# kyutai-labs/pocket-tts

Measured on AMD Instinct MI355X. Metric: audio-seconds/sec (xRT), 100M en model, whole job over all GPUs, higher is better.
Workload: dtype f32

## Files before the change

### include/ptts.h

```cpp
#ifndef PTTS_H_
#define PTTS_H_

#include <stdint.h>

#ifdef __cplusplus
extern "C" {
#endif

#define PTTS_ABI_VERSION 1

typedef struct ptts_engine ptts_engine;
typedef struct ptts_lm_state ptts_lm_state;
typedef struct ptts_mimi_state ptts_mimi_state;
typedef struct ptts_graph ptts_graph;
typedef struct ptts_resampler ptts_resampler;
typedef struct ptts_stretcher ptts_stretcher;

typedef struct ptts_config {
  int32_t d_model, num_heads, num_layers, ff_dim, ldim;
  int32_t flow_dim, flow_depth;
  float max_period;
  int32_t m_dim, m_heads, m_layers, m_ff, m_context;
  float m_max_period;
  int32_t n_filters, ratios[3], kernel_size, res_kernel_size, last_kernel_size, compress;
// ... 109 lines not shown
int ptts_copy_to_host_async(ptts_engine *e, void *h_dst, const void *d_src, int64_t bytes, void *stream);
int ptts_timer_start(ptts_engine *e, void *stream);
int ptts_timer_stop_ms(ptts_engine *e, void *stream, float *h_ms);
int64_t ptts_debug_read(ptts_engine *e, void *state, int32_t is_mimi, const char *name, float *d_out,
                        int64_t capacity, int32_t *rows, int32_t *cols, void *stream);
typedef struct ptts_gemm_case {
  int32_t M, N, C, ntaps;
  int32_t T, xstride, halo, halo_mode;
  int32_t wfmt, pre, epi, act;
  int32_t cfg;
  int32_t krot, lds_target;
  const float *x, *x_prev;
  const float *w, *bias;
  const float *ln_w, *ln_b;
  const float *prevec;
  const float *mod_shift, *mod_scale;
  const float *r, *g, *ls;
  float *y;
  float *w_eff, *w_eff_lo;
  float *ln_s, *ln_c;
  char *label;
  int32_t label_cap;
  int32_t cfg_used;
} ptts_gemm_case;
int ptts_debug_gemm(ptts_engine *e, ptts_gemm_case *c, void *stream);
typedef struct ptts_codec_gemm_case {
  int32_t M, N, C, ntaps;
  int32_t T, halo, par;
  int32_t fmt, kind, pre, epi, act, cfg;
  int32_t mode, cout, stride;
  int32_t yf8, H, Tq, ring, cap;
  float xs, yinv;
  const float *x, *x_prev;
  const float *w, *bias, *ln_w, *ln_b;
  const float *r, *ls;
  const int32_t *offset;
  float *y, *yraw, *y_i16;
  float *x_eff, *xp_eff;
  float *w_eff, *wscale;
  float *ln_s, *ln_c, *rope;
  char *label;
  int32_t label_cap;
  int32_t cfg_used;
} ptts_codec_gemm_case;
int ptts_debug_codec_gemm(ptts_engine *e, ptts_codec_gemm_case *c, void *stream);
typedef struct ptts_attn_case {
// ... 26 lines not shown
```

### pocket_tts_amd/_lib.py

```python

from __future__ import annotations

import ctypes as C
import os
import subprocess
from pathlib import Path

PKG = Path(__file__).resolve().parent
LIB_PATH = PKG / "libptts.so"
SRC = PKG / "csrc" / "ptts.hip"
HEADER = PKG.parent / "include" / "ptts.h"

HIPCC_FLAGS = ["--offload-arch=gfx950", "-O3", "-std=c++17", "-ffp-contract=on", "-Wno-unused-value", "-Wno-unused-result",
               "-shared", "-fPIC"]


class PttsConfig(C.Structure):
    _fields_ = [
        ("d_model", C.c_int32), ("num_heads", C.c_int32), ("num_layers", C.c_int32), ("ff_dim", C.c_int32),
        ("ldim", C.c_int32), ("flow_dim", C.c_int32), ("flow_depth", C.c_int32), ("max_period", C.c_float),
        ("m_dim", C.c_int32), ("m_heads", C.c_int32), ("m_layers", C.c_int32), ("m_ff", C.c_int32),
        ("m_context", C.c_int32), ("m_max_period", C.c_float),
        ("n_filters", C.c_int32), ("ratios", C.c_int32 * 3), ("kernel_size", C.c_int32),
        ("res_kernel_size", C.c_int32), ("last_kernel_size", C.c_int32), ("compress", C.c_int32),
        ("upsample_stride", C.c_int32),
    ]


class PttsTensor(C.Structure):
    _fields_ = [("name", C.c_char_p), ("d_data", C.c_void_p), ("numel", C.c_int64)]


class PttsGemmCase(C.Structure):
    _fields_ = [
        *[(f, C.c_int32) for f in ("M", "N", "C", "ntaps", "T", "xstride", "halo", "halo_mode", "wfmt", "pre", "epi", "act",
                                   "cfg", "krot", "lds_target")],
        *[(f, C.c_void_p) for f in ("x", "x_prev", "w", "bias", "ln_w", "ln_b", "prevec", "mod_shift", "mod_scale", "r", "g",
                                    "ls", "y", "w_eff", "w_eff_lo", "ln_s", "ln_c")],
        ("label", C.c_void_p), ("label_cap", C.c_int32), ("cfg_used", C.c_int32),
    ]


class PttsCodecGemmCase(C.Structure):
    _fields_ = [
        *[(f, C.c_int32) for f in ("M", "N", "C", "ntaps", "T", "halo", "par", "fmt", "kind", "pre", "epi", "act", "cfg",
                                   "mode", "cout", "stride", "yf8", "H", "Tq", "ring", "cap")],
        ("xs", C.c_float), ("yinv", C.c_float),
        *[(f, C.c_void_p) for f in ("x", "x_prev", "w", "bias", "ln_w", "ln_b", "r", "ls", "offset", "y", "yraw", "y_i16",
                                    "x_eff", "xp_eff", "w_eff", "wscale", "ln_s", "ln_c", "rope", "label")],
        ("label_cap", C.c_int32), ("cfg_used", C.c_int32),
    ]


class PttsAttnCase(C.Structure):
    _fields_ = [
        *[(f, C.c_int32) for f in ("B", "Tq", "H", "T", "cap", "ring", "ctx", "splits", "h16", "layer", "n_pre", "pre_T",
                                   "pre_cap", "cascade", "kernel")],
        ("poison_k", C.c_float), ("poison_v", C.c_float),
        *[(f, C.c_void_p) for f in ("q", "k", "v", "pk", "pv", "offset", "pre_len", "pre_id", "y", "label")],
        ("label_cap", C.c_int32), ("kernel_used", C.c_int32), ("splits_used", C.c_int32),
    ]

# ... 165 lines not shown
```

### pocket_tts_amd/csrc/ptts.hip

```cpp
#include "ptts_host.h"
#include "ptts_flow.h"
#include "ptts_bf16.h"
#include "ptts_lm.h"

#include <algorithm>
#include <array>
#include <cmath>
#include <cstdio>
#include <cstring>

static thread_local std::string g_err;
int fail(int code, const std::string &msg) {
  g_err = msg;
  return code;
}
static thread_local std::string g_launch_err;
bool launch_err_pending() { return !g_launch_err.empty(); }
int take_launch_err() {
  std::string m;
  m.swap(g_launch_err);
  return fail(-4, m);
}
void note_launch_err(const std::string &msg) { if (g_launch_err.empty()) g_launch_err = msg; }

// ... 1719 lines not shown

extern "C" void ptts_mimi_state_destroy(ptts_mimi_state *s) {
  if (!s) return;
  hipSetDevice(s->e->device);
  hipDeviceSynchronize();
  hipFree(s->frame); hipFree(s->offset); hipFree(s->kv); hipFree(s->zl); hipFree(s->zq); hipFree(s->u0);
  hipFree(s->u); hipFree(s->h); hipFree(s->ao); hipFree(s->ff); hipFree(s->q); hipFree(s->part);
  hipFree(s->tr_out); hipFree(s->a0); hipFree(s->pcm_dbg); hipFree(s->pcm_part); hipFree(s->pcm_carry); hipFree(s->rope);
  for (int i = 0; i < 3; ++i) { hipFree(s->cbuf[i]); hipFree(s->craw[i]); hipFree(s->rbuf[i]); hipFree(s->sbuf[i]); }
  delete s;
}

extern "C" int ptts_mimi_state_reset(ptts_mimi_state *s, void *stream) {
  hipStream_t st = S(s->e, stream);
  HIPCHK(hipMemsetAsync(s->frame, 0, sizeof(int), st));
  HIPCHK(hipMemsetAsync(s->offset, 0, s->B * sizeof(int), st));
  HIPCHK(hipMemsetAsync(s->zq, 0, (size_t)2 * s->zq_stride * 4, st));
  HIPCHK(hipMemsetAsync(s->tr_out, 0, (size_t)2 * s->tr_stride * 4, st));
  HIPCHK(hipMemsetAsync(s->a0, 0, (size_t)2 * s->a0_stride * 4, st));
  for (int i = 0; i < 3; ++i) {
    HIPCHK(hipMemsetAsync(s->cbuf[i], 0, (size_t)2 * s->c_stride[i] * 4, st));
    HIPCHK(hipMemsetAsync(s->sbuf[i], 0, (size_t)2 * s->s_stride[i] * 4, st));
  }
  HIPCHK(hipMemsetAsync(s->kv, 0, (size_t)s->e->cfg.m_layers * 2 * s->kv_plane() * 4, st));
  if (s->pcm_carry) HIPCHK(hipMemsetAsync(s->pcm_carry, 0, (size_t)2 * s->pcm_cstride * 4, st));
  s->h_frame = 0;
  return 0;
}

extern "C" int ptts_mimi_state_reset_row(ptts_mimi_state *s, int32_t row, void *stream) {
  if (!s || row < 0 || row >= s->B) return fail(-1, "reset_row: row out of range");
  hipStream_t st = S(s->e, stream);
  const int CF = s->e->cfg.m_dim / 16;
  const bool h16 = s->e->codec_bf16, f8 = s->e->codec_fp8;
  const int e_tr = h16 ? 2 : 4, e_a0 = f8 ? 1 : h16 ? 2 : 4;
  set_int_kernel<<<1, 64, 0, st>>>(s->offset + row, 1, 0);
  auto zero_block = [&](float *buf, long stride_floats, int par, int esz) -> hipError_t {
    const size_t per_seq = (size_t)stride_floats / s->B;
    return hipMemsetAsync((char *)buf + (size_t)par * stride_floats * 4 + (size_t)row * per_seq * esz, 0, per_seq * esz, st);
  };
  for (int par = 0; par < 2; ++par) {
    zero_row_fm_kernel<<<cdiv(CF * 16, 256), 256, 0, st>>>(s->zq + par * s->zq_stride, CF, row);
    HIPCHK(zero_block(s->tr_out, s->tr_stride, par, e_tr));
    HIPCHK(zero_block(s->a0, s->a0_stride, par, e_a0));
    for (int i = 0; i < 3; ++i) {
      HIPCHK(zero_block(s->cbuf[i], s->c_stride[i], par, e_a0));
      HIPCHK(zero_block(s->sbuf[i], s->s_stride[i], par, (f8 && i == 2) ? 2 : e_a0));
// ... 755 lines not shown
```

### pocket_tts_amd/csrc/ptts_debug.hip

```cpp
#include "ptts_bf16.h"
#include "ptts_host.h"

#include <algorithm>
#include <cstring>


static constexpr unsigned kDbgUnwritten = 0x7fc00000u;
static constexpr unsigned kDbgGuard = 0x7fa5a5a5u;
static constexpr long kDbgGuardFloats = 16384;
static constexpr long kAttnGuard = 16 * 64;

static __global__ void dbg_guard_kernel(const unsigned *p, long n, unsigned pattern, int *bad) {
  const long i = (long)blockIdx.x * blockDim.x + threadIdx.x;
  if (i < n && p[i] != pattern) atomicOr(bad, 1);
}
__device__ __forceinline__ float dbg_e4m3(uint8_t b) { return __builtin_amdgcn_cvt_f32_fp8((int)b, 0); }
static __global__ void dbg_from_codec_kernel(const void *src, float *dst, int M, int N, int KB, int fmt) {
  const long i = (long)blockIdx.x * blockDim.x + threadIdx.x;
  if (i >= (long)M * N) return;
  const int m = i / N, n = i - (long)m * N;
  const size_t o = fmh_off(m, n & ~3, KB) + (n & 3);
  dst[i] = fmt == 0 ? (float)((const __bf16 *)src)[o] : dbg_e4m3(((const uint8_t *)src)[o]);
}

// ... 104 lines not shown
  const long i = (long)blockIdx.x * blockDim.x + threadIdx.x;
  if (i >= (long)M * N) return;
  const int m = i / N, n = i - (long)m * N;
  dst[i] = src[(((size_t)(m >> 4) * NF + (n >> 4)) * 64 + 16 * ((n & 15) >> 2) + (m & 15)) * 4 + (n & 3)];
}
static __global__ void dbg_unpack_weight_kernel(const void *img, const float *scale, int fmt, float *dst, int N, int KF) {
  const long K = (long)KF * 16;
  const long i = (long)blockIdx.x * blockDim.x + threadIdx.x;
  if (i >= (long)N * K) return;
  const int n = i / K, k = i - (long)n * K;
  const int nt = n >> 4, kf = k >> 4, j = k & 3, lane = 16 * ((k & 15) >> 2) + (n & 15);
  float v;
  if (fmt == 0) v = ((const float *)img)[(((size_t)nt * KF + kf) * 64 + lane) * 4 + j];
  else if (fmt == 1) v = ((float)((const uint8_t *)img)[(size_t)nt * KF * 256 + (size_t)(kf >> 2) * 1024 + lane * 16 + 4 * (kf & 3) + j] - 128.f) * scale[n];
  else v = (float)((const __bf16 *)img)[(((size_t)nt * (KF / 2) + (kf >> 1)) * 64 + lane) * 8 + (kf & 1) * 4 + j];
  dst[i] = v;
}

static int debug_gemm(ptts_engine *e, ptts_gemm_case *c, hipStream_t st, ptts_engine &scr) {
  const int M = c->M, N = c->N, C = c->C, ntaps = c->ntaps, pre = c->pre;
  c->cfg_used = -1;
  if (!c->x || !c->w || !c->y) return fail(-1, "debug_gemm: x, w and y are required");
  if (M < 1 || N < 1 || C < 16 || C % 16 || ntaps < 1) return fail(-1, "debug_gemm: bad shape");
  if (c->wfmt < 0 || c->wfmt > 3 || pre < PRE_NONE || pre > PRE_LNMOD || c->epi < EPI_STORE || c->epi > EPI_GATE ||
      c->act < ACT_NONE || c->act > ACT_ELU || c->cfg < -1 || c->cfg >= kNumCfg)
    return fail(-1, "debug_gemm: enumeration out of range");
  if (c->lds_target < 0 || c->lds_target > 64 * 1024) return fail(-1, "debug_gemm: lds_target above 64 KB");
  int rows_in = M;
  if (ntaps > 1) {
    if (c->T < 16 || c->T % 16 || M % c->T || c->xstride < 1 || c->halo < 0 || c->halo > c->T * c->xstride ||
        ntaps - 1 - c->halo >= c->xstride || c->halo_mode < 0 || c->halo_mode > 2 || (c->halo_mode == 0 && !c->x_prev))
      return fail(-1, "debug_gemm: bad convolution geometry");
    if (pre == PRE_LNFOLD || pre == PRE_LNMOD || pre == PRE_ADDSILU) return fail(-1, "debug_gemm: per-channel prologues are for Linear layers");
    rows_in = M * c->xstride;
  } else if (c->xstride != 1) {
    return fail(-1, "debug_gemm: a Linear has xstride 1");
  }
  if ((pre == PRE_LNFOLD && (!c->ln_w || !c->ln_b)) || (pre == PRE_ADDSILU && !c->prevec) ||
      (pre == PRE_LNMOD && (!c->mod_shift || !c->mod_scale || !c->ln_w != !c->ln_b)))
    return fail(-1, "debug_gemm: missing prologue operand");
  if ((c->epi == EPI_RES && !c->r) || (c->epi == EPI_GATE && (!c->r || !c->g))) return fail(-1, "debug_gemm: missing epilogue operand");
  if (c->wfmt >= 2 && (C / 16) * ntaps % 2) return fail(-1, "debug_gemm: bf16 images need an even number of k-fragments");

  const ptts_tensor tw{"w", c->w, (int64_t)N * C * ntaps}, tb{"b", c->bias, N}, tg{"ln_w", c->ln_w, C}, tbe{"ln_b", c->ln_b, C};
  scr.tmap["w"] = &tw;
  if (c->bias) scr.tmap["b"] = &tb;
  if (pre == PRE_LNFOLD) { scr.tmap["ln_w"] = &tg; scr.tmap["ln_b"] = &tbe; }
  Lin L;
  const bool fold = pre == PRE_LNFOLD;
  CHK(pack_lin(&scr, &L, {{"w", c->bias ? "b" : "", N}}, C, ntaps, 0, 0, 0, fold ? "ln_w" : "", fold ? "ln_b" : "", 0,
// ... 18 lines not shown
    CHK(dallocT(&scr, out, (size_t)pad));
    HIPCHK(hipMemcpyAsync(*out, src, (size_t)n * 4, hipMemcpyDeviceToDevice, st));
    return 0;
  };
  const long yfl = (long)MT * NT * 256;
  float *yfm = nullptr;
  CHK(dallocT(&scr, &yfm, yfl + kDbgGuardFloats));
  HIPCHK(hipMemsetD32Async((hipDeviceptr_t)yfm, (int)kDbgUnwritten, yfl, st));
  HIPCHK(hipMemsetD32Async((hipDeviceptr_t)(yfm + yfl), (int)kDbgGuard, kDbgGuardFloats, st));

  GemmArgs a = mk_gemm(L, xfm, CF, MT, M);
  if (c->wfmt == 3) { a.Wq = (const uint8_t *)L.wsh; a.W = (const float *)L.wsl; a.wfmt = 3; }
  a.Xdstride = xfl;
  a.T = ntaps > 1 ? c->T : 16;
  a.xstride = c->xstride;
  a.halo = c->halo;
  a.halo_mode = c->halo_mode;
  a.zeros = e->zeros;
  a.krot = c->krot;
  a.epi = c->epi;
  a.act = c->act;
  a.Y = yfm;
  a.YF = NT;
  float *tmp = nullptr;
  if (pre == PRE_ADDSILU) { CHK(copy_pad(c->prevec, C, C, &tmp)); a.prevec = tmp; }
  if (pre == PRE_LNMOD) {
    if (c->ln_w) {
      CHK(copy_pad(c->ln_w, C, C, &tmp)); a.lnm_w = tmp;
      CHK(copy_pad(c->ln_b, C, C, &tmp)); a.lnm_b = tmp;
    }
    CHK(to_fm(c->mod_shift, M, C, MT, CF, &tmp)); a.mod_shift = tmp;
    CHK(to_fm(c->mod_scale, M, C, MT, CF, &tmp)); a.mod_scale = tmp;
    a.modF = CF;
  }
  if (c->epi == EPI_RES || c->epi == EPI_GATE) { CHK(to_fm(c->r, M, N, MT, NT, &tmp)); a.R = tmp; a.RF = NT; }
  if (c->epi == EPI_GATE) { CHK(to_fm(c->g, M, N, MT, NT, &tmp)); a.G = tmp; a.GF = NT; }
  if (c->epi == EPI_RES && c->ls) { CHK(copy_pad(c->ls, N, NT * 16, &tmp)); a.ls = tmp; }

  KnobScope knobs(c->lds_target, c->krot);
  int cfg = c->cfg;
  if (cfg >= 0 ? !(pre_supported(a.wfmt, pre) && cfg_valid(cfg, a, pre)) : (cfg = choose_cfg(st, a, pre)) < 0) {
    HIPCHK(hipStreamSynchronize(st));
    return 1;
  }
  std::string label;
  launch_gemm_cfg(st, a, pre, cfg, &label);
  LAUNCHCHK();
  c->cfg_used = cfg;
  put_label(label, c->label, c->label_cap);
  dbg_from_fm_kernel<<<cdiv((long)M * N, 256), 256, 0, st>>>(yfm, c->y, M, N, NT);
  const long nk = (long)N * L.KF * 16;
  if (c->w_eff) {
    if (c->wfmt == 0) dbg_unpack_weight_kernel<<<cdiv(nk, 256), 256, 0, st>>>(L.w, nullptr, 0, c->w_eff, N, L.KF);
    else if (c->wfmt == 1) dbg_unpack_weight_kernel<<<cdiv(nk, 256), 256, 0, st>>>(L.wq, L.wscale, 1, c->w_eff, N, L.KF);
    else dbg_unpack_weight_kernel<<<cdiv(nk, 256), 256, 0, st>>>(c->wfmt == 2 ? L.wb16 : L.wsh, nullptr, 2, c->w_eff, N, L.KF);
  }
  if (c->w_eff_lo && c->wfmt == 3) dbg_unpack_weight_kernel<<<cdiv(nk, 256), 256, 0, st>>>(L.wsl, nullptr, 2, c->w_eff_lo, N, L.KF);
  if (fold && c->ln_s) HIPCHK(hipMemcpyAsync(c->ln_s, L.ln_s, (size_t)N * 4, hipMemcpyDeviceToDevice, st));
  if (fold && c->ln_c) HIPCHK(hipMemcpyAsync(c->ln_c, L.ln_c, (size_t)N * 4, hipMemcpyDeviceToDevice, st));
  return check_guards(scr, st, {yfm + yfl}, kDbgGuardFloats, "debug_gemm: " + label + " wrote past its output");
}

extern "C" int ptts_debug_gemm(ptts_engine *e, ptts_gemm_case *c, void *stream) {
  if (!e || !c) return fail(-1, "debug_gemm: null argument");
  return run_case(e, stream, [&](hipStream_t st, ptts_engine &scr) { return debug_gemm(e, c, st, scr); });
}


static __global__ void dbg_attn_q_kernel(const float *q, float *Q, int B, int Tq, int H, int QB, float poison) {
  const long i = (long)blockIdx.x * blockDim.x + threadIdx.x;
  if (i >= (long)B * H * QB * 1024) return;
  const int j = i & 3, lane = (i >> 2) & 63, df = (i >> 8) & 3;
  const long r = i >> 10;
// ... 384 lines not shown
```

### pocket_tts_amd/csrc/ptts_dispatch.hip

```cpp
#include "ptts_host.h"
#include "ptts_bf16.h"

#include <algorithm>
#include <cstdio>
#include <cstring>

template <int TN, int TM, int WK, int WN, int WM>
static void launch_cfg_q8(hipStream_t st, const GemmArgs &a, int pre) {
  dim3 grid(cdiv(a.NT, TN * WN), cdiv(a.MT, TM * WM));
  dim3 block(64 * WK * WN * WM);
  if (pre == PRE_LNFOLD) gemm_kernel<TN, TM, WK, WN, WM, PRE_LNFOLD, true><<<grid, block, 0, st>>>(a);
  else gemm_kernel<TN, TM, WK, WN, WM, PRE_NONE, true><<<grid, block, 0, st>>>(a);
}

static thread_local int g_lds_target = 0;
static unsigned lds_pad(int static_bytes) { return g_lds_target > static_bytes ? (unsigned)(g_lds_target - static_bytes) : 0u; }
#define LDS_LAUNCH(kernel, grid, block, dyn, st, arg) (kernel)<<<(grid), (block), (dyn), (st)>>>(arg)

template <int TN, int TM, int WK, int WN, int WM>
static void launch_cfg(hipStream_t st, const GemmArgs &a, int pre) {
  dim3 grid(cdiv(a.NT, TN * WN), cdiv(a.MT, TM * WM), pre == PRE_ADDSILU_ROW ? std::max(1, a.row_nz) : 1);
  dim3 block(64 * WK * WN * WM);
  const unsigned dyn = lds_pad(WK > 1 ? WK * WN * WM * TN * TM * 1024 : 0);
  switch (pre) {
    case PRE_NONE: LDS_LAUNCH((gemm_kernel<TN, TM, WK, WN, WM, PRE_NONE>), grid, block, dyn, st, a); break;
    case PRE_LNFOLD: LDS_LAUNCH((gemm_kernel<TN, TM, WK, WN, WM, PRE_LNFOLD>), grid, block, dyn, st, a); break;
    case PRE_LNMOD: LDS_LAUNCH((gemm_kernel<TN, TM, WK, WN, WM, PRE_LNMOD>), grid, block, dyn, st, a); break;
    case PRE_ELU: LDS_LAUNCH((gemm_kernel<TN, TM, WK, WN, WM, PRE_ELU>), grid, block, dyn, st, a); break;
    case PRE_ADDSILU_ROW: LDS_LAUNCH((gemm_kernel<TN, TM, WK, WN, WM, PRE_ADDSILU_ROW>), grid, block, dyn, st, a); break;
    case PRE_LNMOD_ROW: LDS_LAUNCH((gemm_kernel<TN, TM, WK, WN, WM, PRE_LNMOD_ROW>), grid, block, dyn, st, a); break;
    default: LDS_LAUNCH((gemm_kernel<TN, TM, WK, WN, WM, PRE_ADDSILU>), grid, block, dyn, st, a); break;
  }
}

template <int BMT, int BNT>
static void launch_lds(hipStream_t st, const GemmArgs &a, int pre) {
  dim3 grid(cdiv(a.NT, BNT), cdiv(a.MT, BMT));
  static const int variant = [] { const char *v = getenv("PTTS_LDS_VARIANT"); return v ? atoi(v) : 1; }();
  if constexpr (BMT == 4 && BNT <= 4) {
    if (variant == 1 && g_lds_target) {
      const unsigned dyn3 = lds_pad(3 * (BMT + BNT) * 2 * 1024);
      if (pre == PRE_LNFOLD) gemm_lds_kernel<BMT, BNT, 2, PRE_LNFOLD, 3><<<grid, 256, dyn3, st>>>(a);
      else if (pre == PRE_ELU) gemm_lds_kernel<BMT, BNT, 2, PRE_ELU, 3><<<grid, 256, dyn3, st>>>(a);
      else gemm_lds_kernel<BMT, BNT, 2, PRE_NONE, 3><<<grid, 256, dyn3, st>>>(a);
      return;
    }
    if (variant == 2 && g_lds_target && a.KF % 4 == 0 && pre != PRE_ELU) {
      const unsigned dyn4 = lds_pad(2 * (BMT + BNT) * 4 * 1024);
      if (pre == PRE_LNFOLD) gemm_lds_kernel<BMT, BNT, 4, PRE_LNFOLD><<<grid, 256, dyn4, st>>>(a);
      else gemm_lds_kernel<BMT, BNT, 4, PRE_NONE><<<grid, 256, dyn4, st>>>(a);
      return;
    }
  }
  const unsigned dyn = lds_pad(2 * (BMT + BNT) * 2 * 1024);
  if (pre == PRE_LNFOLD) LDS_LAUNCH((gemm_lds_kernel<BMT, BNT, 2, PRE_LNFOLD>), grid, dim3(256), dyn, st, a);
  else if (pre == PRE_ELU) LDS_LAUNCH((gemm_lds_kernel<BMT, BNT, 2, PRE_ELU>), grid, dim3(256), dyn, st, a);
  else LDS_LAUNCH((gemm_lds_kernel<BMT, BNT, 2, PRE_NONE>), grid, dim3(256), dyn, st, a);
}

static int pick_cfg(const GemmArgs &a) {
  const long tiled = (long)cdiv(a.NT, 4) * cdiv(a.MT, 8);
  if (a.MT >= 256 && a.NT >= 4 && a.KF % 2 == 0 && a.epi != EPI_QKV && !a.mod_scale) return a.NT >= 8 ? 8 : 9;
  if (a.MT > 4 && tiled >= 192) return a.NT >= 4 ? 3 : a.NT >= 2 ? 4 : 5;
  if (a.MT >= 8 && a.NT >= 2 && a.KF >= 32 && (long)cdiv(a.NT, 2) * cdiv(a.MT, 4) >= 128) return 7;
  if (a.MT > 64) {
    if (tiled < 192) return 6;
    return a.NT >= 4 ? 3 : a.NT >= 2 ? 4 : 5;
  }
  int tm = a.MT >= 4 ? 4 : a.MT >= 2 ? 2 : 1;
  while (tm > 1 && (long)a.NT * cdiv(a.MT, tm) < 256) tm >>= 1;
  return tm == 4 ? 2 : tm == 2 ? 1 : 0;
}
static const char *const kCfgName[kNumCfg] = {
    "gemm<1,1,8,1,1>", "gemm<1,2,4,1,1>", "gemm<1,4,4,1,1>", "gemm<2,4,1,2,2>", "gemm<2,4,1,1,4>", "gemm<1,4,1,1,4>",
    "gemm<1,1,1,1,4>", "gemm<2,4,4,1,1>", "gemm_lds<4,8,2>", "gemm_lds<4,4,2>", "gemm<2,2,4,1,1>", "gemm<1,1,4,1,1>",
    "gemm_lds<4,2,2>", "gemm<1,2,1,2,2>", "gemm<2,4,2,2,1>", "gemm_lds<8,8,2>", "gemm_lds<8,4,2>", "gemm_lds<8,2,2>"};
static const int kCfgShape[kNumCfg][5] = {{1, 1, 8, 1, 1}, {1, 2, 4, 1, 1}, {1, 4, 4, 1, 1}, {2, 4, 1, 2, 2}, {2, 4, 1, 1, 4},
                                          {1, 4, 1, 1, 4}, {1, 1, 1, 1, 4}, {2, 4, 4, 1, 1}, {8, 4, 0, 0, 0}, {4, 4, 0, 0, 0},
                                          {2, 2, 4, 1, 1}, {1, 1, 4, 1, 1}, {2, 4, 0, 0, 0}, {1, 2, 1, 2, 2}, {2, 4, 2, 2, 1},
                                          {8, 8, 0, 0, 0}, {4, 8, 0, 0, 0}, {2, 8, 0, 0, 0}};

static bool q8_cfg(int cfg) { return cfg == 0 || cfg == 1 || cfg == 2 || cfg == 3 || cfg == 7 || cfg == 10 || cfg == 11; }
static bool b16_cfg(int cfg) { return cfg != 0 && q8_cfg(cfg); }

bool cfg_valid(int cfg, const GemmArgs &a, int pre) {
  const int *s = kCfgShape[cfg];
  if (a.wfmt == 3) {
    if (!split_cfg(cfg) || (pre != PRE_NONE && pre != PRE_LNFOLD)) return false;
    if (a.KF % (2 * s[2])) return false;
  } else if (a.wfmt) {
    if (!(a.wfmt == 2 ? b16_cfg(cfg) : q8_cfg(cfg)) || (pre != PRE_NONE && pre != PRE_LNFOLD)) return false;
    if (a.KF % ((a.wfmt == 1 ? 4 : 2) * s[2])) return false;
  }
  if (s[2] == 0) {
    if (a.KF % 2 || (pre != PRE_NONE && pre != PRE_LNFOLD && pre != PRE_ELU)) return false;
    return a.MT >= s[1] && 2 * a.NT >= s[0];
  }
  const int tn = s[0] * s[3], tm = s[1] * s[4];
  if (tm > 1 && tm > 2 * a.MT) return false;
  if (tn > 1 && tn > 2 * a.NT) return false;
  if (s[2] > 1 && a.KF < 2) return false;
  return true;
}

static int swz_for(int cfg, const GemmArgs &a) {
  static const int swz_env = [] { const char *v = getenv("PTTS_SWZ"); return v ? atoi(v) : -1; }();
  const int *sh = kCfgShape[cfg];
  const int gx = sh[2] == 0 ? cdiv(a.NT, sh[0]) : cdiv(a.NT, sh[0] * sh[3]);
  if (gx <= 1) return 0;
  return swz_env >= 0 ? swz_env : ((double)a.M * a.CF > (double)a.NT * 16 * a.KF && a.MT >= 64);
}

static void launch_by_cfg(hipStream_t st, const GemmArgs &a_in, int pre, int cfg) {
  GemmArgs a = a_in;
  a.swz = swz_for(cfg, a);
  if (a.wfmt == 2) {
    launch_gemm_b16(st, a, pre, cfg, 0);
    return;
  }
  if (a.wfmt == 3) {
    const int *sh = kCfgShape[cfg];
    launch_gemm_split(st, a, pre, cfg, lds_pad(sh[2] > 1 ? sh[2] * sh[3] * sh[4] * sh[0] * sh[1] * 1024 : 0));
// ... 9 lines not shown
      case 11: launch_cfg_q8<1, 1, 4, 1, 1>(st, a, pre); break;
      default: launch_cfg_q8<2, 4, 1, 2, 2>(st, a, pre); break;
    }
    return;
  }
  switch (cfg) {
    case 0: launch_cfg<1, 1, 8, 1, 1>(st, a, pre); break;
    case 1: launch_cfg<1, 2, 4, 1, 1>(st, a, pre); break;
    case 2: launch_cfg<1, 4, 4, 1, 1>(st, a, pre); break;
    case 3: launch_cfg<2, 4, 1, 2, 2>(st, a, pre); break;
    case 4: launch_cfg<2, 4, 1, 1, 4>(st, a, pre); break;
    case 5: launch_cfg<1, 4, 1, 1, 4>(st, a, pre); break;
    case 6: launch_cfg<1, 1, 1, 1, 4>(st, a, pre); break;
    case 7: launch_cfg<2, 4, 4, 1, 1>(st, a, pre); break;
    case 8: launch_lds<4, 8>(st, a, pre); break;
    case 9: launch_lds<4, 4>(st, a, pre); break;
    case 10: launch_cfg<2, 2, 4, 1, 1>(st, a, pre); break;
    case 11: launch_cfg<1, 1, 4, 1, 1>(st, a, pre); break;
    case 12: launch_lds<4, 2>(st, a, pre); break;
    case 13: launch_cfg<1, 2, 1, 2, 2>(st, a, pre); break;
    case 14: launch_cfg<2, 4, 2, 2, 1>(st, a, pre); break;
    case 16: launch_lds<8, 4>(st, a, pre); break;
    case 17: launch_lds<8, 2>(st, a, pre); break;
    default: launch_lds<8, 8>(st, a, pre); break;
  }
}

static constexpr int kTuneVersion = 2;
static thread_local bool g_use_split = false;
static thread_local Tuner *g_tuner = nullptr;
static thread_local const float *g_zeros = nullptr;
static thread_local int g_krot = 1;
KnobScope::KnobScope(int lds_target, int k_rotate, bool use_split) : lds(g_lds_target), krot(g_krot), split(g_use_split) {
  g_krot = k_rotate; g_use_split = use_split; g_lds_target = lds_target;
}
KnobScope::~KnobScope() { g_lds_target = lds; g_use_split = split; g_krot = krot; }
void bind_dispatch(const ptts_engine *e) {
  g_zeros = e->zeros;
  g_tuner = e->tuner;
  g_krot = e->opt_k_rotate;
}
void unbind_dispatch(const ptts_engine *e) {
  if (g_tuner == e->tuner) g_tuner = nullptr;
}

static TuneKey tune_key(const GemmArgs &a, int pre) {
// ... 401 lines not shown
```

### pocket_tts_amd/csrc/ptts_host.h

```cpp
#pragma once
#include "ptts_kernels.h"
#include "ptts_ext.h"

#include <array>
#include <map>
#include <mutex>
#include <string>
#include <vector>

#include "../../include/ptts.h"

#pragma GCC visibility push(hidden)

int fail(int code, const std::string &msg);
#define HIPCHK(x)                                                                                      \
  do {                                                                                                 \
    hipError_t e_ = (x);                                                                               \
    if (e_ != hipSuccess)                                                                              \
      return fail(-2, std::string(#x) + ": " + hipGetErrorString(e_) + " @" + std::to_string(__LINE__)); \
  } while (0)
#define CHK(x)            \
  do {                    \
    int r_ = (x);         \
    if (r_ < 0) return r_; \
// ... 193 lines not shown
  size_t kv_plane() const { return (size_t)B * e->cfg.m_heads * e->ring * 64; }
  float *K(int l) { return kv + (size_t)(2 * l) * kv_plane(); }
  float *V(int l) { return kv + (size_t)(2 * l + 1) * kv_plane(); }
};

hipStream_t S(ptts_engine *e, void *stream);
void bind_engine(ptts_engine *e);
struct AllocScope {
  hipStream_t prev;
  explicit AllocScope(hipStream_t st);
  ~AllocScope();
};
int dalloc(ptts_engine *e, void **p, size_t bytes);
template <typename T>
static int dallocT(ptts_engine *e, T **p, size_t n) {
  return dalloc(e, (void **)p, n * sizeof(T));
}
struct PackPart { std::string w, b; int N; };
int pack_lin(ptts_engine *e, Lin *L, const std::vector<PackPart> &parts, int C, int ntaps, int mode = 0, int cout = 0,
             int stride = 0, const std::string &ln_w = "", const std::string &ln_b = "", int creal = 0, int wfmt = 0);
int pack_lin_h(ptts_engine *e, Lin *L, const std::string &wname, int N, int C, int ntaps, int mode = 0, int cout = 0,
               int stride = 0, const std::string &ln_w = "");

constexpr int kNumCfg = 18;
struct KnobScope {
  int lds, krot;
  bool split;
  KnobScope(int lds_target, int k_rotate, bool use_split = false);
  ~KnobScope();
};
void bind_dispatch(const ptts_engine *e);
void unbind_dispatch(const ptts_engine *e);
bool pre_supported(int wfmt, int pre);
bool cfg_valid(int cfg, const GemmArgs &a, int pre);
int choose_cfg(hipStream_t st, const GemmArgs &a, int pre);
void launch_gemm_cfg(hipStream_t st, const GemmArgs &a, int pre, int cfg, std::string *label = nullptr);
GemmArgs mk_gemm(const Lin &L, const float *X, int XF, int MT, int M);
void launch_gemm(hipStream_t st, const GemmArgs &a_in, int pre);
bool resblock_fusable(const Lin &A, const Lin &Bl, int MT);
void launch_resblock(hipStream_t st, GemmArgs a, const Lin &Bl, int pre = PRE_NONE);

struct AttnKernelInfo { int family, nw, pw, depth, ns, code; const char *name; };
constexpr int kNumAttn = 17;
extern const AttnKernelInfo kAttn[kNumAttn];
int attn_splits(int base, int max_tiles);
bool attn_valid(int k, const AttnArgs &a);
int choose_attn(const AttnArgs &a, int BH, int cascade);
int launch_attention(hipStream_t st, const AttnArgs &at, int BH, int cascade, int kernel, double bytes, double flops,
                     std::string *label = nullptr);

int choose_h_tile(const GemmArgs &a);
GemmArgs gemm_h_args(const GemmArgs &a_in, int pre, const Lin &L);
void launch_h_tile(hipStream_t st, const GemmArgs &a, int pre, int cfg, std::string *label = nullptr);
void launch_gemm_h(hipStream_t st, const GemmArgs &a_in, int pre, const Lin &L);
void launch_f8_tile(hipStream_t st, const GemmArgs &g, int cfg, std::string *label = nullptr);

#pragma GCC visibility pop
// ... 1 lines not shown
```

### pocket_tts_amd/csrc/ptts_kernels.h

```cpp
#pragma once
#include <hip/hip_runtime.h>
#include <stdint.h>
#include <type_traits>

typedef float f32x4 __attribute__((ext_vector_type(4)));
typedef int i32x4 __attribute__((ext_vector_type(4)));

typedef __bf16 bf16x8 __attribute__((ext_vector_type(8)));
typedef __bf16 bf16x4 __attribute__((ext_vector_type(4)));
__device__ __forceinline__ bf16x4 to_bf16x4(f32x4 v) { return __builtin_convertvector(v, bf16x4); }
__device__ __forceinline__ f32x4 from_bf16x4(bf16x4 v) { return __builtin_convertvector(v, f32x4); }
__device__ __forceinline__ size_t fmh_off(size_t row, int n0, int KB) {
  return (((row >> 4) * KB + (n0 >> 5)) * 64 + (((n0 & 31) >> 3) * 16 + (row & 15))) * 8 + (n0 & 7);
}

__device__ __forceinline__ unsigned to_f8x4(f32x4 v) {
  v.x = fminf(fmaxf(v.x, -448.f), 448.f); v.y = fminf(fmaxf(v.y, -448.f), 448.f);
  v.z = fminf(fmaxf(v.z, -448.f), 448.f); v.w = fminf(fmaxf(v.w, -448.f), 448.f);
  int r = __builtin_amdgcn_cvt_pk_fp8_f32(v.x, v.y, 0, false);
  r = __builtin_amdgcn_cvt_pk_fp8_f32(v.z, v.w, r, true);
  return (unsigned)r;
}

#ifndef PTTS_ABLATE
// ... 243 lines not shown
      } else {
        v = (f32x4){0.f, 0.f, 0.f, 0.f};
      }
      *(f32x4 *)(a.Y + (((size_t)mt * a.YF + nt) * 64 + lane) * 4) = v;
    } break;
    case EPI_CONVTR: {
      const int j = n0 / a.cout;
      const int n = n0 - j * a.cout;
      const size_t mo = (size_t)m * a.stride + j;
      const size_t idx = (((mo >> 4) * a.YF + (n >> 4)) * 64 + 16 * g + (mo & 15)) * 4;
      if (a.Yraw) *(f32x4 *)(a.Yraw + par * a.Yrawdstride + idx) = acc;
      float *y = a.Y + par * a.Ydstride;
      *(f32x4 *)(y + idx) = act4(acc, a.act);
    } break;
    case EPI_PCM: {
      if (g == 0 && m < a.M) {
        a.pcm[m] = acc.x;
        if (a.pcm_i16) a.pcm_i16[m] = (int16_t)(fminf(fmaxf(acc.x, -1.0f), 1.0f) * 32767.0f);
      }
    } break;
  }
}

template <int TN, int TM, int WK, int WN, int WM, int PRE_, int WF = 0>
__global__ __launch_bounds__(64 * WK * WN * WM) void gemm_kernel(GemmArgs a) {
  constexpr bool ROWLAT = PRE_ == PRE_LNMOD_ROW;
  constexpr int PRE = ROWLAT ? PRE_LNMOD : PRE_;
  if constexpr (PTTS_ABLATE & 128) return;
  STAMP(0);
  constexpr bool Q8 = WF == 1;
  constexpr bool SPL = WF == 3;
  constexpr bool B16 = WF == 2 || SPL;
  constexpr int NW = WK * WN * WM;
  const int lane = threadIdx.x & 63;
  const int wave = threadIdx.x >> 6;
  const int wk = wave % WK;
  const int wn = (wave / WK) % WN;
  const int wm = wave / (WK * WN);
  int bx, by;
  tile_of_block(a.swz, bx, by);
  const int nt0 = (bx * WN + wn) * TN;
  const int mt0 = (by * WM + wm) * TM;
  const int par = a.par ? (*a.par & 1) : 0;
  const float *Xc = a.X + par * a.Xdstride;
  const float *Xp = a.X + (par ^ 1) * a.Xdstride;
  const int k0 = (a.KF * wk) / WK, k1 = (a.KF * (wk + 1)) / WK;

// ... 125 lines not shown
      xrow[j] = Xc + (((size_t)mtc[j] * a.XF) * 64 + lane) * 4;
      xz[j] = false;
      return;
    }
    const int ts = tin[j] * a.xstride + tp - halo;
    const float *src = Xc;
    long rr = (long)bT[j] * a.xstride + ts;
    if (ts < 0) {
      if (a.halo_mode == 0) { src = Xp; rr += (long)a.T * a.xstride; }
      else if (a.halo_mode == 2) rr = (long)bT[j] * a.xstride;
    }
    xrow[j] = src + (((size_t)(rr >> 4) * a.XF) * 64 + (lane & 48) + (rr & 15)) * 4;
    xz[j] = ts < 0 && a.halo_mode == 1;
  };
#pragma unroll
  for (int j = 0; j < TM; ++j) row_base(j, tap);
#ifndef PTTS_KSPLIT_DIV
#define PTTS_KSPLIT_DIV 2
#endif
  constexpr int U00 = (TN * TM == 1) ? 8 : (TN * TM == 2 && WK > 1) ? 8 : (TN * TM <= 4 && WK > 1) ? 4 : 2;
#ifndef PTTS_KSPLIT_DIV1
#define PTTS_KSPLIT_DIV1 PTTS_KSPLIT_DIV
#endif
  constexpr int KDIV = (TN * TM == 1) ? PTTS_KSPLIT_DIV1 : PTTS_KSPLIT_DIV;
  constexpr int U0 = (WK > 1) ? (U00 / KDIV >= 1 ? U00 / KDIV : 1) : U00;
  constexpr int U = (Q8 && U0 < 4) ? 4 : (B16 && U0 < 2) ? 2 : U0;
  auto load_chunk = [&](auto uc, int kf, f32x4 (*w)[TN], f32x4 (*x)[TM]) {
    constexpr int UU = decltype(uc)::value;
    if (a.ntaps == 1) cf = kf;
#pragma unroll
    for (int u = 0; u < UU; ++u) {
#pragma unroll
      for (int i = 0; i < TN; ++i) {
        if constexpr (PTTS_ABLATE & 2) w[u][i] = (f32x4){1.f, 2.f, 3.f, (float)lane};
        else if constexpr (Q8) {
          if (u % 4 == 0) {
            const i32x4 raw = __builtin_nontemporal_load((const i32x4 *)(wqb[i] + (size_t)(kf + u) * 256));
            w[u / 4][i] = __builtin_bit_cast(f32x4, raw);
          }
        } else if constexpr (B16) {
          if (u % 2 == 0) {
            if constexpr (WK > 1) {
              w[u / 2][i] = __builtin_bit_cast(f32x4, __builtin_nontemporal_load((const i32x4 *)(wqb[i] + (size_t)((kf + u) >> 1) * 1024)));
              if constexpr (SPL)
                w[UU / 2 + u / 2][i] = __builtin_bit_cast(f32x4, __builtin_nontemporal_load((const i32x4 *)((const uint8_t *)wb[i] + (size_t)((kf + u) >> 1) * 1024)));
            } else {
              w[u / 2][i] = *(const f32x4 *)(wqb[i] + (size_t)((kf + u) >> 1) * 1024);
              if constexpr (SPL) w[UU / 2 + u / 2][i] = *(const f32x4 *)((const uint8_t *)wb[i] + (size_t)((kf + u) >> 1) * 1024);
            }
          }
        } else if constexpr (WK > 1) w[u][i] = __builtin_nontemporal_load((const f32x4 *)(wb[i] + (size_t)(kf + u) * 256));
        else w[u][i] = *(const f32x4 *)(wb[i] + (size_t)(kf + u) * 256);
      }
      if constexpr (PTTS_ABLATE & 1) {
#pragma unroll
        for (int j = 0; j < TM; ++j) x[u][j] = (f32x4){1.f, (float)lane, 3.f, (float)kf};
      } else {
#pragma unroll
        for (int j = 0; j < TM; ++j) {
          const float *ptr = xz[j] ? a.zeros : xrow[j] + (size_t)cf * 256;
          x[u][j] = *(const f32x4 *)ptr;
        }
        if (++cf == a.CF) {
          cf = 0;
          ++tap;
#pragma unroll
          for (int j = 0; j < TM; ++j) row_base(j, tap);
        }
      }
    }
  };
  auto compute_chunk = [&](auto uc, int kf, f32x4 (*w)[TN], f32x4 (*x)[TM]) {
    constexpr int UU = decltype(uc)::value;
#pragma unroll
// ... 1732 lines not shown
```

### pocket_tts_amd/engine.py

```python

from __future__ import annotations

import ctypes as C
import numbers
import os
import weakref

import numpy as np
import torch

from . import _lib
from .config import Config
from .weights import mimi_encode_spec, state_dict_spec


def _ptr(t: torch.Tensor | None):
    return None if t is None else C.c_void_p(t.data_ptr())


def make_ptts_config(cfg: Config) -> _lib.PttsConfig:
    t, m, sn = cfg.flow_lm.transformer, cfg.mimi.transformer, cfg.mimi.seanet
    if len(sn.ratios) != 3:
        raise ValueError("SEANet decoder with 3 upsampling stages expected")
    pc = _lib.PttsConfig()
# ... 638 lines not shown
    def mimi_decode(self, state: MimiState, latent: torch.Tensor, out_pcm=None) -> torch.Tensor:
        B = state.batch
        if out_pcm is None:
            out_pcm = torch.empty((B, self.frame_samples), dtype=torch.float32, device=self.device)
        self._pre()
        _lib.check(self.lib.ptts_mimi_decode(self.handle, state.handle, _ptr(latent), _ptr(out_pcm), self._sp))
        latent.record_stream(self.stream)
        out_pcm.record_stream(self.stream)
        self._post()
        return out_pcm

    def debug_read(self, state, name: str) -> torch.Tensor:
        is_mimi = isinstance(state, MimiState)
        cap = 64 * 1024 * 1024
        buf = torch.empty((cap,), dtype=torch.float32, device=self.device)
        self._pre()
        r, c = C.c_int32(), C.c_int32()
        n = self.lib.ptts_debug_read(self.handle, state.handle, int(is_mimi), name.encode(), _ptr(buf), cap,
                                     C.byref(r), C.byref(c), self._sp)
        _lib.check(int(n))
        self.sync()
        return buf[: r.value * c.value].view(r.value, c.value).clone()

    _GEMM_INTS = ("T", "xstride", "halo", "halo_mode", "wfmt", "pre", "epi", "act", "cfg", "krot", "lds_target")
    _GEMM_INS = ("x_prev", "bias", "ln_w", "ln_b", "prevec", "mod_shift", "mod_scale", "r", "g", "ls")

    def debug_gemm(self, x: torch.Tensor, w: torch.Tensor, *, want_weights: bool = False, **kw):
        w3 = w if w.dim() == 3 else w.unsqueeze(2)
        N, Cin, ntaps = w3.shape
        c = _lib.PttsGemmCase()
        c.xstride, c.cfg, c.T = 1, -1, 16
        for k in self._GEMM_INTS:
            if k in kw:
                setattr(c, k, int(kw[k]))
        c.C, c.N, c.ntaps = Cin, N, ntaps
        c.M = x.shape[0] // c.xstride if ntaps > 1 else x.shape[0]
        keep = {}

        def dev(t):
            t = t.to(self.device, torch.float32).contiguous()
            keep[id(t)] = t
            return t.data_ptr()

        c.x, c.w = dev(x), dev(w3)
        for k in self._GEMM_INS:
            if kw.get(k) is not None:
                setattr(c, k, dev(kw[k]))
# ... 367 lines not shown
```

Baseline: 5967.

## Add GEMM tile configs, temporal weight loads for multi-row grids, drop KV reset

Adds three new GEMM tile configurations, one of them with a fixed K-split divisor, so the autotuner has more candidates. Weight loads in K-split kernels now use ordinary cached loads instead of nontemporal ones whenever more than one row block runs, so weights can be reused across row blocks through cache. The full KV-cache memset in the mimi state reset is removed to cut per-reset memory traffic, which relies on the cache contents being masked by the offsets. The debug GEMM path gains transposed-conv support and can force configs on any row count.

```diff
diff --git a/include/ptts.h b/include/ptts.h
--- a/include/ptts.h
+++ b/include/ptts.h
@@ -155,6 +155,7 @@
   char *label;
   int32_t label_cap;
   int32_t cfg_used;
+  int32_t cout;
 } ptts_gemm_case;
 int ptts_debug_gemm(ptts_engine *e, ptts_gemm_case *c, void *stream);
 typedef struct ptts_codec_gemm_case {
diff --git a/pocket_tts_amd/_lib.py b/pocket_tts_amd/_lib.py
--- a/pocket_tts_amd/_lib.py
+++ b/pocket_tts_amd/_lib.py
@@ -37,7 +37,7 @@
                                    "cfg", "krot", "lds_target")],
         *[(f, C.c_void_p) for f in ("x", "x_prev", "w", "bias", "ln_w", "ln_b", "prevec", "mod_shift", "mod_scale", "r", "g",
                                     "ls", "y", "w_eff", "w_eff_lo", "ln_s", "ln_c")],
-        ("label", C.c_void_p), ("label_cap", C.c_int32), ("cfg_used", C.c_int32),
+        ("label", C.c_void_p), ("label_cap", C.c_int32), ("cfg_used", C.c_int32), ("cout", C.c_int32),
     ]
 
 
diff --git a/pocket_tts_amd/csrc/ptts.hip b/pocket_tts_amd/csrc/ptts.hip
--- a/pocket_tts_amd/csrc/ptts.hip
+++ b/pocket_tts_amd/csrc/ptts.hip
@@ -1765,7 +1765,6 @@
     HIPCHK(hipMemsetAsync(s->cbuf[i], 0, (size_t)2 * s->c_stride[i] * 4, st));
     HIPCHK(hipMemsetAsync(s->sbuf[i], 0, (size_t)2 * s->s_stride[i] * 4, st));
   }
-  HIPCHK(hipMemsetAsync(s->kv, 0, (size_t)s->e->cfg.m_layers * 2 * s->kv_plane() * 4, st));
   if (s->pcm_carry) HIPCHK(hipMemsetAsync(s->pcm_carry, 0, (size_t)2 * s->pcm_cstride * 4, st));
   s->h_frame = 0;
   return 0;
diff --git a/pocket_tts_amd/csrc/ptts_debug.hip b/pocket_tts_amd/csrc/ptts_debug.hip
--- a/pocket_tts_amd/csrc/ptts_debug.hip
+++ b/pocket_tts_amd/csrc/ptts_debug.hip
@@ -150,10 +150,12 @@
   c->cfg_used = -1;
   if (!c->x || !c->w || !c->y) return fail(-1, "debug_gemm: x, w and y are required");
   if (M < 1 || N < 1 || C < 16 || C % 16 || ntaps < 1) return fail(-1, "debug_gemm: bad shape");
-  if (c->wfmt < 0 || c->wfmt > 3 || pre < PRE_NONE || pre > PRE_LNMOD || c->epi < EPI_STORE || c->epi > EPI_GATE ||
+  if (c->wfmt < 0 || c->wfmt > 3 || pre < PRE_NONE || pre > PRE_LNMOD || c->epi < EPI_STORE || (c->epi > EPI_GATE && c->epi != EPI_CONVTR) ||
       c->act < ACT_NONE || c->act > ACT_ELU || c->cfg < -1 || c->cfg >= kNumCfg)
     return fail(-1, "debug_gemm: enumeration out of range");
   if (c->lds_target < 0 || c->lds_target > 64 * 1024) return fail(-1, "debug_gemm: lds_target above 64 KB");
+  if (c->epi == EPI_CONVTR && (ntaps != 2 || c->xstride != 1 || c->halo != 1 || c->cout < 16 || c->cout % 16 || N % c->cout))
+    return fail(-1, "debug_gemm: a transposed conv has 2 taps, halo 1 and N = stride * cout with cout % 16 == 0");
   int rows_in = M;
   if (ntaps > 1) {
     if (c->T < 16 || c->T % 16 || M % c->T || c->xstride < 1 || c->halo < 0 || c->halo > c->T * c->xstride ||
@@ -218,6 +220,7 @@
   a.act = c->act;
   a.Y = yfm;
   a.YF = NT;
+  if (c->epi == EPI_CONVTR) { a.cout = c->cout; a.stride = N / c->cout; a.YF = c->cout / 16; }
   float *tmp = nullptr;
   if (pre == PRE_ADDSILU) { CHK(copy_pad(c->prevec, C, C, &tmp)); a.prevec = tmp; }
   if (pre == PRE_LNMOD) {
@@ -235,7 +238,7 @@
 
   KnobScope knobs(c->lds_target, c->krot);
   int cfg = c->cfg;
-  if (cfg >= 0 ? !(pre_supported(a.wfmt, pre) && cfg_valid(cfg, a, pre)) : (cfg = choose_cfg(st, a, pre)) < 0) {
+  if (cfg >= 0 ? !(pre_supported(a.wfmt, pre) && cfg_valid(cfg, a, pre, cfg >= 18)) : (cfg = choose_cfg(st, a, pre)) < 0) {
     HIPCHK(hipStreamSynchronize(st));
     return 1;
   }
@@ -244,7 +247,8 @@
   LAUNCHCHK();
   c->cfg_used = cfg;
   put_label(label, c->label, c->label_cap);
-  dbg_from_fm_kernel<<<cdiv((long)M * N, 256), 256, 0, st>>>(yfm, c->y, M, N, NT);
+  if (c->epi == EPI_CONVTR) dbg_from_fm_kernel<<<cdiv((long)M * N, 256), 256, 0, st>>>(yfm, c->y, M * a.stride, a.cout, a.YF);
+  else dbg_from_fm_kernel<<<cdiv((long)M * N, 256), 256, 0, st>>>(yfm, c->y, M, N, NT);
   const long nk = (long)N * L.KF * 16;
   if (c->w_eff) {
     if (c->wfmt == 0) dbg_unpack_weight_kernel<<<cdiv(nk, 256), 256, 0, st>>>(L.w, nullptr, 0, c->w_eff, N, L.KF);
diff --git a/pocket_tts_amd/csrc/ptts_dispatch.hip b/pocket_tts_amd/csrc/ptts_dispatch.hip
--- a/pocket_tts_amd/csrc/ptts_dispatch.hip
+++ b/pocket_tts_amd/csrc/ptts_dispatch.hip
@@ -17,20 +17,31 @@
 static unsigned lds_pad(int static_bytes) { return g_lds_target > static_bytes ? (unsigned)(g_lds_target - static_bytes) : 0u; }
 #define LDS_LAUNCH(kernel, grid, block, dyn, st, arg) (kernel)<<<(grid), (block), (dyn), (st)>>>(arg)
 
-template <int TN, int TM, int WK, int WN, int WM>
-static void launch_cfg(hipStream_t st, const GemmArgs &a, int pre) {
+template <int TN, int TM, int WK, int WN, int WM, bool WNT, int KD = 0>
+static void launch_cfg_w(hipStream_t st, const GemmArgs &a, int pre) {
   dim3 grid(cdiv(a.NT, TN * WN), cdiv(a.MT, TM * WM), pre == PRE_ADDSILU_ROW ? std::max(1, a.row_nz) : 1);
   dim3 block(64 * WK * WN * WM);
   const unsigned dyn = lds_pad(WK > 1 ? WK * WN * WM * TN * TM * 1024 : 0);
   switch (pre) {
-    case PRE_NONE: LDS_LAUNCH((gemm_kernel<TN, TM, WK, WN, WM, PRE_NONE>), grid, block, dyn, st, a); break;
-    case PRE_LNFOLD: LDS_LAUNCH((gemm_kernel<TN, TM, WK, WN, WM, PRE_LNFOLD>), grid, block, dyn, st, a); break;
-    case PRE_LNMOD: LDS_LAUNCH((gemm_kernel<TN, TM, WK, WN, WM, PRE_LNMOD>), grid, block, dyn, st, a); break;
-    case PRE_ELU: LDS_LAUNCH((gemm_kernel<TN, TM, WK, WN, WM, PRE_ELU>), grid, block, dyn, st, a); break;
-    case PRE_ADDSILU_ROW: LDS_LAUNCH((gemm_kernel<TN, TM, WK, WN, WM, PRE_ADDSILU_ROW>), grid, block, dyn, st, a); break;
-    case PRE_LNMOD_ROW: LDS_LAUNCH((gemm_kernel<TN, TM, WK, WN, WM, PRE_LNMOD_ROW>), grid, block, dyn, st, a); break;
-    default: LDS_LAUNCH((gemm_kernel<TN, TM, WK, WN, WM, PRE_ADDSILU>), grid, block, dyn, st, a); break;
-  }
+    case PRE_NONE: LDS_LAUNCH((gemm_kernel<TN, TM, WK, WN, WM, PRE_NONE, 0, WNT, KD>), grid, block, dyn, st, a); break;
+    case PRE_LNFOLD: LDS_LAUNCH((gemm_kernel<TN, TM, WK, WN, WM, PRE_LNFOLD, 0, WNT, KD>), grid, block, dyn, st, a); break;
+    case PRE_LNMOD: LDS_LAUNCH((gemm_kernel<TN, TM, WK, WN, WM, PRE_LNMOD, 0, WNT, KD>), grid, block, dyn, st, a); break;
+    case PRE_ELU: LDS_LAUNCH((gemm_kernel<TN, TM, WK, WN, WM, PRE_ELU, 0, WNT, KD>), grid, block, dyn, st, a); break;
+    case PRE_ADDSILU_ROW: LDS_LAUNCH((gemm_kernel<TN, TM, WK, WN, WM, PRE_ADDSILU_ROW, 0, WNT, KD>), grid, block, dyn, st, a); break;
+    case PRE_LNMOD_ROW: LDS_LAUNCH((gemm_kernel<TN, TM, WK, WN, WM, PRE_LNMOD_ROW, 0, WNT, KD>), grid, block, dyn, st, a); break;
+    default: LDS_LAUNCH((gemm_kernel<TN, TM, WK, WN, WM, PRE_ADDSILU, 0, WNT, KD>), grid, block, dyn, st, a); break;
+  }
+}
+template <int TN, int TM, int WK, int WN, int WM>
+static void launch_cfg(hipStream_t st, const GemmArgs &a, int pre) {
+  if constexpr (WK > 1 && TM >= 4) {
+    static const bool all_nt = [] { const char *v = getenv("PTTS_W_NT"); return v && atoi(v) != 0; }();
+    if (cdiv(a.MT, TM * WM) > 1 && !all_nt) {
+      launch_cfg_w<TN, TM, WK, WN, WM, false>(st, a, pre);
+      return;
+    }
+  }
+  launch_cfg_w<TN, TM, WK, WN, WM, true>(st, a, pre);
 }
 
 template <int BMT, int BNT>
@@ -74,16 +85,17 @@
 static const char *const kCfgName[kNumCfg] = {
     "gemm<1,1,8,1,1>", "gemm<1,2,4,1,1>", "gemm<1,4,4,1,1>", "gemm<2,4,1,2,2>", "gemm<2,4,1,1,4>", "gemm<1,4,1,1,4>",
     "gemm<1,1,1,1,4>", "gemm<2,4,4,1,1>", "gemm_lds<4,8,2>", "gemm_lds<4,4,2>", "gemm<2,2,4,1,1>", "gemm<1,1,4,1,1>",
-    "gemm_lds<4,2,2>", "gemm<1,2,1,2,2>", "gemm<2,4,2,2,1>", "gemm_lds<8,8,2>", "gemm_lds<8,4,2>", "gemm_lds<8,2,2>"};
+    "gemm_lds<4,2,2>", "gemm<1,2,1,2,2>", "gemm<2,4,2,2,1>", "gemm_lds<8,8,2>", "gemm_lds<8,4,2>", "gemm_lds<8,2,2>",
+    "gemm<1,8,4,1,1>", "gemm<1,4,1,2,2>", "gemm<2,4,4,1,1>x2"};
 static const int kCfgShape[kNumCfg][5] = {{1, 1, 8, 1, 1}, {1, 2, 4, 1, 1}, {1, 4, 4, 1, 1}, {2, 4, 1, 2, 2}, {2, 4, 1, 1, 4},
                                           {1, 4, 1, 1, 4}, {1, 1, 1, 1, 4}, {2, 4, 4, 1, 1}, {8, 4, 0, 0, 0}, {4, 4, 0, 0, 0},
                                           {2, 2, 4, 1, 1}, {1, 1, 4, 1, 1}, {2, 4, 0, 0, 0}, {1, 2, 1, 2, 2}, {2, 4, 2, 2, 1},
-                                          {8, 8, 0, 0, 0}, {4, 8, 0, 0, 0}, {2, 8, 0, 0, 0}};
+                                          {8, 8, 0, 0, 0}, {4, 8, 0, 0, 0}, {2, 8, 0, 0, 0}, {1, 8, 4, 1, 1}, {1, 4, 1, 2, 2}, {2, 4, 4, 1, 1}};
 
 static bool q8_cfg(int cfg) { return cfg == 0 || cfg == 1 || cfg == 2 || cfg == 3 || cfg == 7 || cfg == 10 || cfg == 11; }
 static bool b16_cfg(int cfg) { return cfg != 0 && q8_cfg(cfg); }
 
-bool cfg_valid(int cfg, const GemmArgs &a, int pre) {
+bool cfg_valid(int cfg, const GemmArgs &a, int pre, bool any_rows) {
   const int *s = kCfgShape[cfg];
   if (a.wfmt == 3) {
     if (!split_cfg(cfg) || (pre != PRE_NONE && pre != PRE_LNFOLD)) return false;
@@ -97,7 +109,7 @@
     return a.MT >= s[1] && 2 * a.NT >= s[0];
   }
   const int tn = s[0] * s[3], tm = s[1] * s[4];
-  if (tm > 1 && tm > 2 * a.MT) return false;
+  if (tm > 1 && tm > 2 * a.MT && !any_rows) return false;
   if (tn > 1 && tn > 2 * a.NT) return false;
   if (s[2] > 1 && a.KF < 2) return false;
   return true;
@@ -153,6 +165,12 @@
     case 14: launch_cfg<2, 4, 2, 2, 1>(st, a, pre); break;
     case 16: launch_lds<8, 4>(st, a, pre); break;
     case 17: launch_lds<8, 2>(st, a, pre); break;
+    case 18: launch_cfg<1, 8, 4, 1, 1>(st, a, pre); break;
+    case 19: launch_cfg<1, 4, 1, 2, 2>(st, a, pre); break;
+    case 20:
+      if (cdiv(a.MT, 4) > 1) launch_cfg_w<2, 4, 4, 1, 1, false, 1>(st, a, pre);
+      else launch_cfg_w<2, 4, 4, 1, 1, true, 1>(st, a, pre);
+      break;
     default: launch_lds<8, 8>(st, a, pre); break;
   }
 }
diff --git a/pocket_tts_amd/csrc/ptts_host.h b/pocket_tts_amd/csrc/ptts_host.h
--- a/pocket_tts_amd/csrc/ptts_host.h
+++ b/pocket_tts_amd/csrc/ptts_host.h
@@ -239,7 +239,7 @@
 int pack_lin_h(ptts_engine *e, Lin *L, const std::string &wname, int N, int C, int ntaps, int mode = 0, int cout = 0,
                int stride = 0, const std::string &ln_w = "");
 
-constexpr int kNumCfg = 18;
+constexpr int kNumCfg = 21;
 struct KnobScope {
   int lds, krot;
   bool split;
@@ -249,7 +249,7 @@
 void bind_dispatch(const ptts_engine *e);
 void unbind_dispatch(const ptts_engine *e);
 bool pre_supported(int wfmt, int pre);
-bool cfg_valid(int cfg, const GemmArgs &a, int pre);
+bool cfg_valid(int cfg, const GemmArgs &a, int pre, bool any_rows = false);
 int choose_cfg(hipStream_t st, const GemmArgs &a, int pre);
 void launch_gemm_cfg(hipStream_t st, const GemmArgs &a, int pre, int cfg, std::string *label = nullptr);
 GemmArgs mk_gemm(const Lin &L, const float *X, int XF, int MT, int M);
diff --git a/pocket_tts_amd/csrc/ptts_kernels.h b/pocket_tts_amd/csrc/ptts_kernels.h
--- a/pocket_tts_amd/csrc/ptts_kernels.h
+++ b/pocket_tts_amd/csrc/ptts_kernels.h
@@ -289,7 +289,7 @@
   }
 }
 
-template <int TN, int TM, int WK, int WN, int WM, int PRE_, int WF = 0>
+template <int TN, int TM, int WK, int WN, int WM, int PRE_, int WF = 0, bool WNT = true, int KD = 0>
 __global__ __launch_bounds__(64 * WK * WN * WM) void gemm_kernel(GemmArgs a) {
   constexpr bool ROWLAT = PRE_ == PRE_LNMOD_ROW;
   constexpr int PRE = ROWLAT ? PRE_LNMOD : PRE_;
@@ -461,7 +461,7 @@
 #ifndef PTTS_KSPLIT_DIV1
 #define PTTS_KSPLIT_DIV1 PTTS_KSPLIT_DIV
 #endif
-  constexpr int KDIV = (TN * TM == 1) ? PTTS_KSPLIT_DIV1 : PTTS_KSPLIT_DIV;
+  constexpr int KDIV = KD > 0 ? KD : (TN * TM == 1) ? PTTS_KSPLIT_DIV1 : PTTS_KSPLIT_DIV;
   constexpr int U0 = (WK > 1) ? (U00 / KDIV >= 1 ? U00 / KDIV : 1) : U00;
   constexpr int U = (Q8 && U0 < 4) ? 4 : (B16 && U0 < 2) ? 2 : U0;
   auto load_chunk = [&](auto uc, int kf, f32x4 (*w)[TN], f32x4 (*x)[TM]) {
@@ -488,7 +488,7 @@
               if constexpr (SPL) w[UU / 2 + u / 2][i] = *(const f32x4 *)((const uint8_t *)wb[i] + (size_t)((kf + u) >> 1) * 1024);
             }
           }
-        } else if constexpr (WK > 1) w[u][i] = __builtin_nontemporal_load((const f32x4 *)(wb[i] + (size_t)(kf + u) * 256));
+        } else if constexpr (WK > 1 && WNT) w[u][i] = __builtin_nontemporal_load((const f32x4 *)(wb[i] + (size_t)(kf + u) * 256));
         else w[u][i] = *(const f32x4 *)(wb[i] + (size_t)(kf + u) * 256);
       }
       if constexpr (PTTS_ABLATE & 1) {
diff --git a/pocket_tts_amd/engine.py b/pocket_tts_amd/engine.py
--- a/pocket_tts_amd/engine.py
+++ b/pocket_tts_amd/engine.py
@@ -684,7 +684,7 @@
         self.sync()
         return buf[: r.value * c.value].view(r.value, c.value).clone()
 
-    _GEMM_INTS = ("T", "xstride", "halo", "halo_mode", "wfmt", "pre", "epi", "act", "cfg", "krot", "lds_target")
+    _GEMM_INTS = ("T", "xstride", "halo", "halo_mode", "wfmt", "pre", "epi", "act", "cfg", "krot", "lds_target", "cout")
     _GEMM_INS = ("x_prev", "bias", "ln_w", "ln_b", "prevec", "mod_shift", "mod_scale", "r", "g", "ls")
 
     def debug_gemm(self, x: torch.Tensor, w: torch.Tensor, *, want_weights: bool = False, **kw):
```

Result: no change. 5944, median of 2 (-0.4%).
